# ray-project/ray

Measured on AMD Instinct MI355X. Metric: train_samples_per_sec, higher is better.
Workload: dtype bf16; 1 GPU; model=llama3-8b, global_batch=8, micro_batch=8, seq_len=4096, parallelism=dp1, n_params=8030261248, bucket_mb=128, grad_checkpoint=False, harness=ray_amd.train.TorchTrainer

## Files before the change

### __graft_entry__.py

```python
from __future__ import annotations

import os
import sys

sys.path.insert(0, os.path.dirname(os.path.abspath(__file__)))


def build() -> None:
    os.environ.setdefault("PYTORCH_ROCM_ARCH", "gfx950")
    from ray_amd.csrc import build as _b

    _b.build(verbose=True)
    import ray_amd
    import ray_amd.ops

    assert os.path.exists(_b.OUT), "HIP extension missing after build"


def smoke() -> None:
    import torch

    from ray_amd.models.llama import CONFIGS, LlamaModel
    from ray_amd.ops import HAVE_HIP_OPS, FusedAdamW

    assert torch.cuda.is_available(), "smoke() needs a GPU"
    assert HAVE_HIP_OPS, "ray_amd HIP extension not loaded"
    dev = torch.device("cuda", 0)
    cfg = CONFIGS["llama-tiny"]
    model = LlamaModel(cfg, dtype=torch.bfloat16).to(dev)
    model.cosT = model.cosT.to(dev)
    model.sinT = model.sinT.to(dev)
    tokens = torch.randint(0, cfg.vocab_size, (2, 128), device=dev)
    targets = torch.randint(0, cfg.vocab_size, (2, 128), device=dev)
    loss = model(tokens, targets)
    loss.backward()
    opt = FusedAdamW(model.parameters(), lr=1e-3)
    opt.step()
    torch.cuda.synchronize()
    print("smoke ok: loss", float(loss.detach().float().cpu()))


if __name__ == "__main__":
    build()
    if "--smoke" in sys.argv:
        smoke()
```

### ray_amd/csrc/ops.hip

```cpp
#include <torch/extension.h>
#include <ATen/hip/HIPContext.h>

#include "hip/rmsnorm.hip"
#include "hip/elementwise.hip"
#include "hip/rl_scans.hip"
#include "hip/cross_entropy.hip"
#include "hip/flash_attn_v5.hip"
#include "hip/flash_attn_v6.hip"
#include "hip/fa_bwd.hip"
#include "hip/fa_bwd_v3.hip"
#include "hip/fa_bwd_v4.hip"
#include "hip/fa_bwd_dq_v4.hip"
#include "hip/fa_bwd_dkv_v5.hip"
#include "hip/fa_bwd_dkv_v6.hip"
#include "hip/fa_bwd_dq_v5.hip"
#include "hip/gemv.hip"
#include "hip/paged_attn.hip"

#define CHECK_IN(x)                                                     \
  TORCH_CHECK(x.is_cuda(), #x " must be on GPU");                       \
  TORCH_CHECK(x.is_contiguous(), #x " must be contiguous")

static inline hipStream_t cur_stream() {
  return at::hip::getCurrentHIPStream().stream();
}

static inline int grid_for(long long n, int block = 256, int cap = 2048) {
  long long g = (n + block - 1) / block;
  return (int)std::min<long long>(g, cap);
}


std::vector<at::Tensor> rmsnorm_fwd(at::Tensor x, at::Tensor w, double eps) {
  CHECK_IN(x);
  CHECK_IN(w);
  TORCH_CHECK(x.scalar_type() == at::kBFloat16, "x must be bf16");
  int H = (int)x.size(-1);
  TORCH_CHECK(H % 8 == 0, "H must be a multiple of 8");
  long long N = x.numel() / H;
  auto y = at::empty_like(x);
  auto inv = at::empty({N}, x.options().dtype(at::kFloat));
  hipLaunchKernelGGL(rmsnorm_fwd_bf16, dim3((unsigned)N), dim3(256), 0,
                     cur_stream(), (const short*)x.data_ptr(),
                     (const short*)w.data_ptr(), (short*)y.data_ptr(),
                     inv.data_ptr<float>(), H, (float)eps);
  return {y, inv};
}

std::vector<at::Tensor> rmsnorm_bwd(at::Tensor dy, at::Tensor x, at::Tensor w,
                                    at::Tensor inv) {
  CHECK_IN(dy); CHECK_IN(x); CHECK_IN(w); CHECK_IN(inv);
  int H = (int)x.size(-1);
  long long N = x.numel() / H;
  auto dx = at::empty_like(x);
  auto dw = at::zeros({H}, x.options().dtype(at::kFloat));
  hipLaunchKernelGGL(rmsnorm_bwd_dx_bf16, dim3((unsigned)N), dim3(256), 0,
                     cur_stream(), (const short*)dy.data_ptr(),
                     (const short*)x.data_ptr(), (const short*)w.data_ptr(),
                     inv.data_ptr<float>(), (short*)dx.data_ptr(), H);
  int row_splits = (int)std::min<long long>(256, std::max<long long>(1, N / 64));
  hipLaunchKernelGGL(rmsnorm_bwd_dw_bf16,
                     dim3((H + 255) / 256, row_splits), dim3(256), 0,
                     cur_stream(), (const short*)dy.data_ptr(),
                     (const short*)x.data_ptr(), inv.data_ptr<float>(),
                     dw.data_ptr<float>(), N, H);
  return {dx, dw};
}


at::Tensor swiglu_fwd(at::Tensor a, at::Tensor b) {
  CHECK_IN(a); CHECK_IN(b);
  TORCH_CHECK(a.numel() == b.numel() && a.numel() % 8 == 0);
  auto y = at::empty_like(a);
  long long n8 = a.numel() / 8;
  hipLaunchKernelGGL(swiglu_fwd_bf16, dim3(grid_for(n8)), dim3(256), 0,
                     cur_stream(), (const short*)a.data_ptr(),
                     (const short*)b.data_ptr(), (short*)y.data_ptr(), n8);
  return y;
}

std::vector<at::Tensor> swiglu_bwd(at::Tensor dy, at::Tensor a, at::Tensor b) {
  CHECK_IN(dy); CHECK_IN(a); CHECK_IN(b);
  auto da = at::empty_like(a);
  auto db = at::empty_like(b);
  long long n8 = a.numel() / 8;
  hipLaunchKernelGGL(swiglu_bwd_bf16, dim3(grid_for(n8)), dim3(256), 0,
                     cur_stream(), (const short*)dy.data_ptr(),
                     (const short*)a.data_ptr(), (const short*)b.data_ptr(),
                     (short*)da.data_ptr(), (short*)db.data_ptr(), n8);
  return {da, db};
}


at::Tensor rope_apply(at::Tensor x, at::Tensor cosT, at::Tensor sinT,
                      int64_t n_heads, int64_t T, int64_t sign) {
  CHECK_IN(cosT); CHECK_IN(sinT);
  int D = (int)x.size(-1);
  long long rows = x.numel() / D;
  long long in_rs = (long long)n_heads * D;
  if (!x.is_contiguous()) {
// ... 120 lines not shown
              "paged_attn: num_splits must be 1..1024");
  auto out = at::empty({B, Hq, D}, q.options());
  at::Tensor ws;
  float *ws_o = nullptr, *ws_ml = nullptr;
  if (S > 1) {
    long long need = (long long)B * Hq * S * (D + 2);
    if (workspace.has_value()) {
      ws = *workspace;
      CHECK_IN(ws);
      TORCH_CHECK(ws.scalar_type() == at::kFloat && ws.numel() >= need,
                  "paged_attn: workspace must be fp32 with >= B*Hq*S*(D+2) "
                  "elements");
    } else {
      ws = at::empty({need}, q.options().dtype(at::kFloat));
    }
    ws_o = ws.data_ptr<float>();
    ws_ml = ws_o + (long long)B * Hq * S * D;
  }
#define PA_LAUNCH(DD, RR)                                                   \
  launch_paged_decode<DD, RR>(q, k_cache, v_cache, block_table, seq_lens,   \
                              out, ws_o, ws_ml, S, Hkv)
#define PA_REP(DD)                                                          \
  switch (rep) {                                                            \
    case 1: PA_LAUNCH(DD, 1); break;                                        \
    case 2: PA_LAUNCH(DD, 2); break;                                        \
    case 4: PA_LAUNCH(DD, 4); break;                                        \
    default: PA_LAUNCH(DD, 8); break;                                       \
  }
  if (D == 64) { PA_REP(64) } else { PA_REP(128) }
#undef PA_REP
#undef PA_LAUNCH
  if (S > 1) launch_paged_reduce(ws, out, B, Hq, D, S);
  return out;
}

static long long paged_row_stride(const at::Tensor& t, const char* name) {
  TORCH_CHECK(t.is_cuda(), name, " must be on GPU");
  TORCH_CHECK(t.scalar_type() == at::kBFloat16, name, " must be bf16");
  TORCH_CHECK(t.dim() == 3 && t.stride(2) == 1 && t.stride(1) == t.size(2),
              name, " must be [B, H, D] with a contiguous [H, D] tail");
  TORCH_CHECK(t.stride(0) % 8 == 0 &&
              reinterpret_cast<uintptr_t>(t.data_ptr()) % 16 == 0,
              name, " rows must be 16-byte aligned");
  return (long long)t.stride(0);
}

at::Tensor rope_append_paged(at::Tensor q, at::Tensor k, at::Tensor v,
                             at::Tensor cosT, at::Tensor sinT, at::Tensor pos,
                             at::Tensor block_table, at::Tensor k_cache,
                             at::Tensor v_cache) {
  long long q_rs = paged_row_stride(q, "q");
  long long k_rs = paged_row_stride(k, "k");
  long long v_rs = paged_row_stride(v, "v");
  CHECK_IN(cosT); CHECK_IN(sinT);
  CHECK_I32(pos);
  CHECK_I32(block_table);
  int B = (int)q.size(0), Hq = (int)q.size(1), D = (int)q.size(2);
  int Hkv = (int)k.size(1);
  TORCH_CHECK(D == 64 || D == 128, "paged_attn: head_dim must be 64 or 128");
  TORCH_CHECK(k.size(0) == B && v.size(0) == B && k.size(2) == D &&
              v.size(2) == D && v.size(1) == Hkv,
              "q/k/v shapes disagree");
  check_paged_cache(k_cache, v_cache, Hkv, D);
  TORCH_CHECK(cosT.scalar_type() == at::kFloat &&
              sinT.scalar_type() == at::kFloat && cosT.dim() == 2 &&
              cosT.size(1) == D / 2 && sinT.sizes() == cosT.sizes(),
              "cosT/sinT must be fp32 [T, D/2]");
  TORCH_CHECK(pos.dim() == 1 && pos.size(0) == B, "pos must be [B]");
  TORCH_CHECK(block_table.dim() == 2 && block_table.size(0) == B &&
              block_table.size(1) >= 1,
              "block_table must be [B, max_pages]");
  auto q_rot = at::empty({B, Hq, D}, q.options());
  if (B == 0) return q_rot;
  hipLaunchKernelGGL(rope_append_paged_bf16, dim3(B), dim3(256), 0,
                     cur_stream(), (const short*)q.data_ptr(),
                     (const short*)k.data_ptr(), (const short*)v.data_ptr(),
                     q_rs, k_rs, v_rs, cosT.data_ptr<float>(),
                     sinT.data_ptr<float>(), pos.data_ptr<int>(),
                     block_table.data_ptr<int>(), (short*)k_cache.data_ptr(),
                     (short*)v_cache.data_ptr(), (short*)q_rot.data_ptr(), Hq,
                     Hkv, D, (int)cosT.size(0), (int)k_cache.size(0),
                     (int)block_table.size(1));
  return q_rot;
}


void adamw_step(at::Tensor p, at::Tensor g, at::Tensor m, at::Tensor v,
                at::Tensor master, double lr, double beta1, double beta2,
                double eps, double wd, int64_t step, double grad_scale) {
  CHECK_IN(p); CHECK_IN(g); CHECK_IN(m); CHECK_IN(v);
  long long n = p.numel();
  float bc1 = 1.f - powf((float)beta1, (float)step);
  float bc2 = 1.f - powf((float)beta2, (float)step);
  if (p.scalar_type() == at::kBFloat16) {
    CHECK_IN(master);
    hipLaunchKernelGGL(adamw_step_bf16, dim3(grid_for(n)), dim3(256), 0,
                       cur_stream(), (short*)p.data_ptr(),
                       (const short*)g.data_ptr(), m.data_ptr<float>(),
                       v.data_ptr<float>(), master.data_ptr<float>(), n,
                       (float)lr, (float)beta1, (float)beta2, (float)eps,
                       (float)wd, bc1, bc2, (float)grad_scale);
  } else {
    hipLaunchKernelGGL(adamw_step_f32, dim3(grid_for(n)), dim3(256), 0,
                       cur_stream(), p.data_ptr<float>(),
                       g.data_ptr<float>(), m.data_ptr<float>(),
                       v.data_ptr<float>(), n, (float)lr, (float)beta1,
                       (float)beta2, (float)eps, (float)wd, bc1, bc2,
                       (float)grad_scale);
  }
}


std::vector<at::Tensor> gae(at::Tensor rewards, at::Tensor values,
                            at::Tensor cont, double gamma, double lam) {
  CHECK_IN(rewards); CHECK_IN(values); CHECK_IN(cont);
  int T = (int)rewards.size(0);
  int B = (int)rewards.size(1);
  TORCH_CHECK(values.size(0) == T + 1, "values must be [T+1, B]");
  auto adv = at::empty_like(rewards);
  auto vt = at::empty_like(rewards);
  hipLaunchKernelGGL(gae_scan_f32, dim3((B + 255) / 256), dim3(256), 0,
                     cur_stream(), rewards.data_ptr<float>(),
                     values.data_ptr<float>(), cont.data_ptr<float>(),
                     adv.data_ptr<float>(), vt.data_ptr<float>(), T, B,
                     (float)gamma, (float)lam);
  return {adv, vt};
}

std::vector<at::Tensor> vtrace(at::Tensor log_rhos, at::Tensor rewards,
                               at::Tensor values, at::Tensor cont,
                               double gamma, double rho_clip, double c_clip,
                               double rho_pg_clip) {
  CHECK_IN(log_rhos); CHECK_IN(rewards); CHECK_IN(values); CHECK_IN(cont);
  int T = (int)rewards.size(0);
  int B = (int)rewards.size(1);
  auto vs = at::empty_like(rewards);
  auto pg = at::empty_like(rewards);
  hipLaunchKernelGGL(vtrace_scan_f32, dim3((B + 255) / 256), dim3(256), 0,
                     cur_stream(), log_rhos.data_ptr<float>(),
                     rewards.data_ptr<float>(), values.data_ptr<float>(),
                     cont.data_ptr<float>(), vs.data_ptr<float>(),
                     pg.data_ptr<float>(), T, B, (float)gamma,
                     (float)rho_clip, (float)c_clip, (float)rho_pg_clip);
  return {vs, pg};
}


at::Tensor img_normalize(at::Tensor in, at::Tensor mean, at::Tensor inv_std) {
  CHECK_IN(in); CHECK_IN(mean); CHECK_IN(inv_std);
  TORCH_CHECK(in.scalar_type() == at::kByte && in.dim() == 4);
  long long N = in.size(0);
  int H = (int)in.size(1), W = (int)in.size(2), C = (int)in.size(3);
  auto out = at::empty({N, C, H, W}, in.options().dtype(at::kBFloat16));
  long long total = in.numel();
  hipLaunchKernelGGL(img_norm_u8_bf16, dim3(grid_for(total)), dim3(256), 0,
                     cur_stream(), in.data_ptr<unsigned char>(),
                     (short*)out.data_ptr(), mean.data_ptr<float>(),
                     inv_std.data_ptr<float>(), N, H, W, C);
  return out;
}


std::vector<at::Tensor> ce_fwd(at::Tensor logits, at::Tensor target) {
  CHECK_IN(logits); CHECK_IN(target);
  TORCH_CHECK(logits.scalar_type() == at::kBFloat16);
  TORCH_CHECK(target.scalar_type() == at::kInt);
// ... 165 lines not shown
    }
    if (v4 && getenv("RAY_AMD_FA_NO_DKV5") == nullptr) {
      hipLaunchKernelGGL(fa_bwd_dkv_v5_bf16, dim3(T / 256, B * Hkv),
                         dim3(512), 0, cur_stream(),
                         (const short*)q.data_ptr(),
                         (const short*)k.data_ptr(),
                         (const short*)v.data_ptr(),
                         (const short*)d_o.data_ptr(), lse.data_ptr<float>(),
                         dsum.data_ptr<float>(), (short*)dk.data_ptr(),
                         (short*)dv.data_ptr(), B, Hq, Hkv, T,
                         causal ? 1 : 0, scale, bthd);
      return {dq, dk, dv};
    }
    if (v4) {
      hipLaunchKernelGGL(fa_bwd_dv_v4_bf16, dim3(T / 256, B * Hkv),
                         dim3(512), 0, cur_stream(),
                         (const short*)q.data_ptr(),
                         (const short*)k.data_ptr(),
                         (const short*)v.data_ptr(),
                         (const short*)d_o.data_ptr(), lse.data_ptr<float>(),
                         (short*)dv.data_ptr(), B, Hq, Hkv, T,
                         causal ? 1 : 0, scale, bthd);
      hipLaunchKernelGGL(fa_bwd_dk_v4_bf16, dim3(T / 256, B * Hkv),
                         dim3(512), 0, cur_stream(),
                         (const short*)q.data_ptr(),
                         (const short*)k.data_ptr(),
                         (const short*)v.data_ptr(),
                         (const short*)d_o.data_ptr(), lse.data_ptr<float>(),
                         dsum.data_ptr<float>(), (short*)dk.data_ptr(), B,
                         Hq, Hkv, T, causal ? 1 : 0, scale, bthd);
      return {dq, dk, dv};
    }
    hipLaunchKernelGGL(fa_bwd_dv_v3_bf16, dim3(T / 128, B * Hkv),
                       dim3(256), 0, cur_stream(),
                       (const short*)q.data_ptr(),
                       (const short*)k.data_ptr(),
                       (const short*)v.data_ptr(),
                       (const short*)d_o.data_ptr(), lse.data_ptr<float>(),
                       (short*)dv.data_ptr(), B, Hq, Hkv, T,
                       causal ? 1 : 0, scale);
    hipLaunchKernelGGL(fa_bwd_dk_v3_bf16, dim3(T / 128, B * Hkv),
                       dim3(256), 0, cur_stream(),
                       (const short*)q.data_ptr(),
                       (const short*)k.data_ptr(),
                       (const short*)v.data_ptr(),
                       (const short*)d_o.data_ptr(), lse.data_ptr<float>(),
                       dsum.data_ptr<float>(), (short*)dk.data_ptr(), B,
                       Hq, Hkv, T, causal ? 1 : 0, scale);
    return {dq, dk, dv};
  }
  if (split) {
    hipLaunchKernelGGL(fa_bwd_dv_bf16, dim3(T / 128, B * Hkv), dim3(256),
                       0, cur_stream(), (const short*)q.data_ptr(),
                       (const short*)k.data_ptr(),
                       (const short*)v.data_ptr(),
                       (const short*)d_o.data_ptr(), lse.data_ptr<float>(),
                       (short*)dv.data_ptr(), B, Hq, Hkv, T,
                       causal ? 1 : 0, scale);
    hipLaunchKernelGGL(fa_bwd_dk_bf16, dim3(T / 128, B * Hkv), dim3(256),
                       0, cur_stream(), (const short*)q.data_ptr(),
                       (const short*)k.data_ptr(),
                       (const short*)v.data_ptr(),
                       (const short*)d_o.data_ptr(), lse.data_ptr<float>(),
                       dsum.data_ptr<float>(), (short*)dk.data_ptr(), B,
                       Hq, Hkv, T, causal ? 1 : 0, scale);
  } else {
    hipLaunchKernelGGL(fa_bwd_dkv_bf16, dim3(T / 128, B * Hkv), dim3(256),
                       0, cur_stream(), (const short*)q.data_ptr(),
                       (const short*)k.data_ptr(),
                       (const short*)v.data_ptr(),
                       (const short*)d_o.data_ptr(), lse.data_ptr<float>(),
                       dsum.data_ptr<float>(), (short*)dk.data_ptr(),
                       (short*)dv.data_ptr(), B, Hq, Hkv, T,
                       causal ? 1 : 0, scale);
  }
  return {dq, dk, dv};
}

PYBIND11_MODULE(TORCH_EXTENSION_NAME, m) {
  m.def("flash_attn_fwd", &flash_attn_fwd);
  m.def("flash_attn_bwd", &flash_attn_bwd);
  m.def("rmsnorm_fwd", &rmsnorm_fwd);
  m.def("gemv", &gemv);
  m.def("paged_attn_decode", &paged_attn_decode, py::arg("q"),
        py::arg("k_cache"), py::arg("v_cache"), py::arg("block_table"),
        py::arg("seq_lens"), py::arg("num_splits"),
        py::arg("workspace") = py::none());
  m.def("paged_attn_reduce", &paged_attn_reduce);
  m.def("rope_append_paged", &rope_append_paged);
  m.def("rmsnorm_bwd", &rmsnorm_bwd);
  m.def("swiglu_fwd", &swiglu_fwd);
  m.def("swiglu_bwd", &swiglu_bwd);
  m.def("rope_apply", &rope_apply);
  m.def("adamw_step", &adamw_step);
  m.def("gae", &gae);
  m.def("vtrace", &vtrace);
  m.def("img_normalize", &img_normalize);
  m.def("ce_fwd", &ce_fwd);
  m.def("ce_bwd", &ce_bwd);
  m.attr("gfx_arch") = "gfx950";
}
```

### ray_amd/models/llama.py

```python
from __future__ import annotations

from dataclasses import dataclass

import os

import torch
import torch.nn as nn
import torch.nn.functional as F

from ray_amd import ops


@dataclass
class LlamaConfig:
    vocab_size: int = 128256
    hidden_size: int = 4096
    intermediate_size: int = 14336
    num_layers: int = 32
    num_heads: int = 32
    num_kv_heads: int = 8
    max_seq_len: int = 8192
    rope_base: float = 500000.0
    rms_eps: float = 1e-5
    tie_embeddings: bool = False


CONFIGS = {
    "llama3-8b": LlamaConfig(),
    "llama3-1b": LlamaConfig(
        hidden_size=2048, intermediate_size=8192, num_layers=16,
        num_heads=32, num_kv_heads=8
    ),
    "llama-tiny": LlamaConfig(
        vocab_size=512, hidden_size=256, intermediate_size=512,
        num_layers=2, num_heads=4, num_kv_heads=2, max_seq_len=512,
    ),
}


class Attention(nn.Module):
    def __init__(self, cfg: LlamaConfig, dtype=torch.bfloat16):
        super().__init__()
        self.cfg = cfg
        self.head_dim = cfg.hidden_size // cfg.num_heads
        self.n_rep = cfg.num_heads // cfg.num_kv_heads
        self._fused_qkv = not os.environ.get("RAY_AMD_NO_FUSED_QKV")
        qd = cfg.num_heads * self.head_dim
        kvd = cfg.num_kv_heads * self.head_dim
        if self._fused_qkv:
            self.qkv_proj = nn.Linear(
                cfg.hidden_size, qd + 2 * kvd, bias=False, dtype=dtype
            )
        else:
            self.q_proj = nn.Linear(
                cfg.hidden_size, qd, bias=False, dtype=dtype)
            self.k_proj = nn.Linear(
                cfg.hidden_size, kvd, bias=False, dtype=dtype)
            self.v_proj = nn.Linear(
                cfg.hidden_size, kvd, bias=False, dtype=dtype)
        self.o_proj = nn.Linear(
            cfg.num_heads * self.head_dim, cfg.hidden_size, bias=False, dtype=dtype
        )

    def qkv(self, x, lin=None):
        B, T, _ = x.shape
        cfg = self.cfg
        hd = self.head_dim
        if self._fused_qkv:
            qkv = (self.qkv_proj(x) if lin is None
                   else lin(x, self.qkv_proj.weight))
            q, k, v = qkv.split(
                [cfg.num_heads * hd, cfg.num_kv_heads * hd,
                 cfg.num_kv_heads * hd], dim=-1)
            return (q.view(B, T, cfg.num_heads, hd),
                    k.view(B, T, cfg.num_kv_heads, hd),
                    v.view(B, T, cfg.num_kv_heads, hd))
        if lin is None:
            return (self.q_proj(x).view(B, T, cfg.num_heads, hd),
                    self.k_proj(x).view(B, T, cfg.num_kv_heads, hd),
                    self.v_proj(x).view(B, T, cfg.num_kv_heads, hd))
        return (lin(x, self.q_proj.weight).view(B, T, cfg.num_heads, hd),
                lin(x, self.k_proj.weight).view(B, T, cfg.num_kv_heads, hd),
                lin(x, self.v_proj.weight).view(B, T, cfg.num_kv_heads, hd))

    def forward(self, x, cosT, sinT, kv_cache=None, pos0: int = 0):
        B, T, H = x.shape
        cfg = self.cfg
        q, k, v = self.qkv(x)
        if self._fused_qkv:
            v = v.contiguous()
        q = ops.rope(q, cosT[pos0 : pos0 + T], sinT[pos0 : pos0 + T])
        k = ops.rope(k, cosT[pos0 : pos0 + T], sinT[pos0 : pos0 + T])
        q = q.transpose(1, 2)
        k = k.transpose(1, 2)
        v = v.transpose(1, 2)
        if kv_cache is not None:
            k, v = kv_cache.update(k, v, pos0)
        is_causal = kv_cache is None or T > 1
        if (
            kv_cache is None
            and q.is_cuda
            and q.dtype == torch.bfloat16
            and self.head_dim == 128
            and T % 128 == 0
            and not os.environ.get("RAY_AMD_ATTN_SDPA")
        ):
            out = ops.flash_attention(q, k, v, causal=True)
        else:
            out = F.scaled_dot_product_attention(
                q, k, v, is_causal=is_causal, enable_gqa=True
            )
        out = out.transpose(1, 2).reshape(B, T, -1)
        return self.o_proj(out)


class MLP(nn.Module):
    def __init__(self, cfg: LlamaConfig, dtype=torch.bfloat16):
        super().__init__()
        self.gate_proj = nn.Linear(
            cfg.hidden_size, cfg.intermediate_size, bias=False, dtype=dtype
        )
        self.up_proj = nn.Linear(
            cfg.hidden_size, cfg.intermediate_size, bias=False, dtype=dtype
        )
        self.down_proj = nn.Linear(
            cfg.intermediate_size, cfg.hidden_size, bias=False, dtype=dtype
        )

    def forward(self, x):
        return self.down_proj(ops.swiglu(self.gate_proj(x), self.up_proj(x)))


class Block(nn.Module):
    def __init__(self, cfg: LlamaConfig, dtype=torch.bfloat16):
        super().__init__()
        self.attn_norm = ops.RMSNorm(cfg.hidden_size, cfg.rms_eps, dtype)
        self.attn = Attention(cfg, dtype)
        self.mlp_norm = ops.RMSNorm(cfg.hidden_size, cfg.rms_eps, dtype)
        self.mlp = MLP(cfg, dtype)

    def forward(self, x, cosT, sinT, kv_cache=None, pos0=0):
        x = x + self.attn(self.attn_norm(x), cosT, sinT, kv_cache, pos0)
        x = x + self.mlp(self.mlp_norm(x))
        return x


class LlamaModel(nn.Module):
    def __init__(self, cfg: LlamaConfig, dtype=torch.bfloat16,
                 gradient_checkpointing: bool = False):
        super().__init__()
        self.cfg = cfg
        self.dtype = dtype
        self.embed = nn.Embedding(cfg.vocab_size, cfg.hidden_size, dtype=dtype)
        self.layers = nn.ModuleList(Block(cfg, dtype) for _ in range(cfg.num_layers))
        self.final_norm = ops.RMSNorm(cfg.hidden_size, cfg.rms_eps, dtype)
        self.lm_head = nn.Linear(
            cfg.hidden_size, cfg.vocab_size, bias=False, dtype=dtype
        )
        if cfg.tie_embeddings:
            self.lm_head.weight = self.embed.weight
        cosT, sinT = ops.rope_tables(
            cfg.max_seq_len, cfg.hidden_size // cfg.num_heads, cfg.rope_base
        )
        self.register_buffer("cosT", cosT, persistent=False)
        self.register_buffer("sinT", sinT, persistent=False)
        self.gradient_checkpointing = gradient_checkpointing
        self.apply(self._init_weights)

    def _init_weights(self, m):
        if isinstance(m, nn.Linear):
            nn.init.normal_(m.weight, std=0.02)
        elif isinstance(m, nn.Embedding):
            nn.init.normal_(m.weight, std=0.02)

    def forward(self, tokens, targets=None, kv_caches=None, pos0: int = 0):
        x = self.embed(tokens)
        for i, layer in enumerate(self.layers):
            cache = kv_caches[i] if kv_caches is not None else None
            if self.gradient_checkpointing and self.training:
                x = torch.utils.checkpoint.checkpoint(
                    layer, x, self.cosT, self.sinT, use_reentrant=False
                )
            else:
                x = layer(x, self.cosT, self.sinT, cache, pos0)
        x = self.final_norm(x)
        if targets is not None:
            if x.is_cuda and os.environ.get("RAY_AMD_CHUNKED_CE"):
                return ops.lm_head_cross_entropy(
                    x.reshape(-1, self.cfg.hidden_size),
                    self.lm_head.weight,
                    targets.reshape(-1),
                )
            logits = self.lm_head(x)
            return ops.cross_entropy(
                logits.view(-1, self.cfg.vocab_size), targets.reshape(-1)
            )
        return self.lm_head(x)

    def num_params(self) -> int:
        return sum(p.numel() for p in self.parameters())


class GraphedDecoder:

    def __init__(self, model: "LlamaModel", batch_size: int, max_T: int,
                 device):
        self.m = model
        cfg = model.cfg
        self.B = batch_size
        self.max_T = max_T
        self.device = device
        hd = cfg.hidden_size // cfg.num_heads
        dt = model.dtype
        self.cache_k = [
            torch.zeros(batch_size, cfg.num_kv_heads, max_T, hd,
                        device=device, dtype=dt)
            for _ in range(cfg.num_layers)
        ]
        self.cache_v = [torch.zeros_like(k) for k in self.cache_k]
        self.in_tok = torch.zeros(batch_size, 1, dtype=torch.long, device=device)
        self.pos = torch.zeros(1, dtype=torch.long, device=device)
        self.mask = torch.full((1, 1, 1, max_T), float("-inf"),
                               device=device, dtype=torch.float32)
        self.out_logits = None
        self.graph = None

    def _step(self):
        m = self.m
        cfg = m.cfg
        B = self.B
        hd = cfg.hidden_size // cfg.num_heads
        x = m.embed(self.in_tok)
        cos = m.cosT.index_select(0, self.pos).view(1, 1, 1, hd // 2)
        sin = m.sinT.index_select(0, self.pos).view(1, 1, 1, hd // 2)
        lin = ops.linear_sb
        for li, layer in enumerate(m.layers):
            h = layer.attn_norm(x)
            at = layer.attn
            q, k, v = at.qkv(h, lin=lin)
# ... 169 lines not shown
```

### ray_amd/ops/__init__.py

```python
from __future__ import annotations

import torch

try:
    from ray_amd import _hip_ops as _K

    HAVE_HIP_OPS = True
except ImportError:
    _K = None
    HAVE_HIP_OPS = False


def _require_ext(name: str):
    if _K is None:
        raise RuntimeError(
            f"ray_amd HIP extension not built but {name} was called on a GPU "
            "tensor. Run `python ray_amd/csrc/build.py`."
        )




def rmsnorm_ref(x: torch.Tensor, w: torch.Tensor, eps: float = 1e-5):
    xf = x.float()
    inv = torch.rsqrt(xf.pow(2).mean(-1, keepdim=True) + eps)
    return (xf * inv * w.float()).to(x.dtype)


class _RMSNorm(torch.autograd.Function):
    @staticmethod
    def forward(ctx, x, w, eps):
        _require_ext("rmsnorm")
        y, inv = _K.rmsnorm_fwd(x.contiguous(), w.contiguous(), eps)
        ctx.save_for_backward(x, w, inv)
        return y

    @staticmethod
    def backward(ctx, dy):
        x, w, inv = ctx.saved_tensors
        dx, dw = _K.rmsnorm_bwd(dy.contiguous(), x, w, inv)
        return dx, dw.to(w.dtype), None


def rmsnorm(x: torch.Tensor, w: torch.Tensor, eps: float = 1e-5):
    if not x.is_cuda:
        xf = x.float()
        inv = torch.rsqrt(xf.pow(2).mean(-1, keepdim=True) + eps)
        return (xf * inv * w.float()).to(x.dtype)
    return _RMSNorm.apply(x, w, eps)


class RMSNorm(torch.nn.Module):
    def __init__(self, dim: int, eps: float = 1e-5, dtype=torch.bfloat16):
        super().__init__()
        self.weight = torch.nn.Parameter(torch.ones(dim, dtype=dtype))
        self.eps = eps

    def forward(self, x):
        return rmsnorm(x, self.weight, self.eps)




def swiglu_ref(a: torch.Tensor, b: torch.Tensor):
    return (torch.nn.functional.silu(a.float()) * b.float()).to(a.dtype)


class _SwiGLU(torch.autograd.Function):
    @staticmethod
    def forward(ctx, a, b):
        _require_ext("swiglu")
        a = a.contiguous()
        b = b.contiguous()
        ctx.save_for_backward(a, b)
        return _K.swiglu_fwd(a, b)

    @staticmethod
    def backward(ctx, dy):
        a, b = ctx.saved_tensors
        da, db = _K.swiglu_bwd(dy.contiguous(), a, b)
        return da, db


def swiglu(a: torch.Tensor, b: torch.Tensor):
    if not a.is_cuda:
        return torch.nn.functional.silu(a) * b
    return _SwiGLU.apply(a, b)




def rope_tables(T: int, D: int, base: float = 500000.0, device="cpu"):
    half = D // 2
    inv_freq = 1.0 / (
        base ** (torch.arange(0, half, dtype=torch.float64) / half)
    )
    t = torch.arange(T, dtype=torch.float64)
    ang = torch.outer(t, inv_freq)
    return (
        ang.cos().float().contiguous().to(device),
        ang.sin().float().contiguous().to(device),
    )


def rope_ref(x: torch.Tensor, cosT: torch.Tensor, sinT: torch.Tensor):
    B, T, Hn, D = x.shape
    half = D // 2
    x1 = x[..., :half].float()
    x2 = x[..., half:].float()
    c = cosT[:T].view(1, T, 1, half)
    s = sinT[:T].view(1, T, 1, half)
    return torch.cat([x1 * c - x2 * s, x2 * c + x1 * s], dim=-1).to(x.dtype)


class _Rope(torch.autograd.Function):
    @staticmethod
    def forward(ctx, x, cosT, sinT, n_heads, T):
        _require_ext("rope")
        ctx.meta = (cosT, sinT, n_heads, T)
        if not (x.dim() == 4 and x.stride(3) == 1
                and x.stride(2) == x.size(3)
                and x.stride(0) == x.size(1) * x.stride(1)):
            x = x.contiguous()
        return _K.rope_apply(x, cosT, sinT, n_heads, T, 1)

    @staticmethod
    def backward(ctx, dy):
        cosT, sinT, n_heads, T = ctx.meta
        dx = _K.rope_apply(dy.contiguous(), cosT, sinT, n_heads, T, -1)
        return dx, None, None, None, None


def rope(x: torch.Tensor, cosT: torch.Tensor, sinT: torch.Tensor):
    B, T, Hn, D = x.shape
    if not x.is_cuda:
        return rope_ref(x, cosT, sinT)
    return _Rope.apply(x, cosT[:T].contiguous(), sinT[:T].contiguous(), Hn, T)


def linear_sb(x: torch.Tensor, weight: torch.Tensor) -> torch.Tensor:
    K = x.shape[-1]
    rows = x.numel() // K
    if (
        _K is not None
        and x.is_cuda
        and x.dtype == torch.bfloat16
        and weight.dtype == torch.bfloat16
        and rows <= 2
        and weight.shape[0] <= 8192
        and K % 512 == 0
        and not torch.is_grad_enabled()
    ):
        y = _K.gemv(x.reshape(rows, K).contiguous(), weight)
        return y.view(*x.shape[:-1], weight.shape[0])
    return torch.nn.functional.linear(x, weight)




def cross_entropy_ref(logits: torch.Tensor, target: torch.Tensor):
    return torch.nn.functional.cross_entropy(
        logits.float(), target.long(), ignore_index=-100, reduction="mean"
    )


class _FusedCE(torch.autograd.Function):
    @staticmethod
    def forward(ctx, logits, target):
        _require_ext("cross_entropy")
        logits = logits.contiguous()
        t32 = target.to(torch.int32).contiguous()
        loss, mx, lse = _K.ce_fwd(logits, t32)
        nvalid = (t32 >= 0).sum().clamp(min=1)
        ctx.save_for_backward(logits, t32, mx, lse, nvalid)
        return loss.sum() / nvalid.float()

    @staticmethod
    def backward(ctx, dloss):
        logits, t32, mx, lse, nvalid = ctx.saved_tensors
        per_row = (dloss / nvalid.float()).expand(logits.size(0)).contiguous()
        dl = _K.ce_bwd(logits, t32, mx, lse, per_row)
        return dl, None


def cross_entropy(logits: torch.Tensor, target: torch.Tensor):
    if not logits.is_cuda:
        return cross_entropy_ref(logits, target)
    return _FusedCE.apply(logits, target)


class _ChunkedLmHeadCE(torch.autograd.Function):

    @staticmethod
    def forward(ctx, x, weight, target, chunk_rows):
        _require_ext("cross_entropy")
        x = x.contiguous()
        t32 = target.to(torch.int32).contiguous()
        N = x.shape[0]
        nvalid = (t32 >= 0).sum().clamp(min=1)
        loss_sum = torch.zeros((), dtype=torch.float32, device=x.device)
        for s in range(0, N, chunk_rows):
            e = min(s + chunk_rows, N)
            logits = (x[s:e] @ weight.t()).contiguous()
            l, mx, lse = _K.ce_fwd(logits, t32[s:e])
            loss_sum += l.sum()
        ctx.save_for_backward(x, weight, t32, nvalid)
        ctx.chunk = chunk_rows
        return loss_sum / nvalid.float()

    @staticmethod
    def backward(ctx, dloss):
        x, w, t32, nvalid = ctx.saved_tensors
        N = x.shape[0]
        chunk = ctx.chunk
        dx = torch.empty_like(x)
        dw_acc = torch.zeros_like(w, dtype=torch.float32)
        scale = dloss / nvalid.float()
        for s in range(0, N, chunk):
            e = min(s + chunk, N)
            logits = (x[s:e] @ w.t()).contiguous()
            _, mx, lse = _K.ce_fwd(logits, t32[s:e])
            per_row = scale.expand(e - s).contiguous()
            dl = _K.ce_bwd(logits, t32[s:e], mx, lse, per_row)
            dx[s:e] = dl @ w
            dw_acc += (dl.t() @ x[s:e]).float()
        return dx, dw_acc.to(w.dtype), None, None


def lm_head_cross_entropy(x: torch.Tensor, weight: torch.Tensor,
                          target: torch.Tensor,
                          chunk_rows: int = 8192) -> torch.Tensor:
    if not x.is_cuda:
        return cross_entropy_ref(x.float() @ weight.t().float(), target)
    return _ChunkedLmHeadCE.apply(x, weight, target, chunk_rows)




# ... 315 lines not shown
```

Measured before the change: 4.818 samples/s.

## Add custom MFMA weight-gradient GEMM kernel and route Linear backward through it

Adds a hand-written HIP bf16 weight-gradient GEMM (dy^T @ x) with 256x256 output tiles, LDS double buffering via global_load_lds, transposed LDS reads, XCD-aware tile scheduling and an optional wave-stagger barrier. A custom autograd Linear routes backward dW through this kernel for a table of Llama-8B shapes. A grouped variant computes the gate and up projection weight gradients in a single launch. It aims to beat the library GEMM on the tall-skinny reduction-over-tokens shape, at the cost of extra launch-shape restrictions and a Python autograd layer around every projection.

```diff
diff --git a/__graft_entry__.py b/__graft_entry__.py
--- a/__graft_entry__.py
+++ b/__graft_entry__.py
@@ -36,6 +36,11 @@
     loss.backward()
     opt = FusedAdamW(model.parameters(), lr=1e-3)
     opt.step()
+    from ray_amd.ops import gemm_wgrad
+    dy = torch.randn(128, 256, device=dev).bfloat16()
+    x = torch.randn(128, 256, device=dev).bfloat16()
+    dw, ref = gemm_wgrad(dy, x).float(), dy.float().t() @ x.float()
+    assert (dw - ref).norm() <= 5e-3 * ref.norm(), "gemm_wgrad mismatch"
     torch.cuda.synchronize()
     print("smoke ok: loss", float(loss.detach().float().cpu()))
 
diff --git a/ray_amd/csrc/hip/gemm_wgrad.hip b/ray_amd/csrc/hip/gemm_wgrad.hip
--- /dev/null
+++ b/ray_amd/csrc/hip/gemm_wgrad.hip
@@ -0,0 +1,243 @@
+#include "common.h"
+#include "fa_bwd_lds_layout.h"
+
+typedef __attribute__((ext_vector_type(8))) __bf16 wg_bf16x8;
+typedef __attribute__((ext_vector_type(16))) float wg_f32x16;
+typedef __attribute__((ext_vector_type(2))) unsigned int wg_u32x2;
+typedef __attribute__((ext_vector_type(4))) unsigned int wg_u32x4;
+
+#define WG_STAGE 65536
+#define WG_HALF 16384
+#define WG_B 32768
+
+template <int OFF>
+DEV_INLINE wg_u32x2 wg_tr(unsigned addr) {
+  wg_u32x2 v;
+  asm volatile("ds_read_b64_tr_b16 %0, %1 offset:%2"
+               : "=v"(v)
+               : "v"(addr), "n"(OFF)
+               : "memory");
+  return v;
+}
+
+DEV_INLINE wg_bf16x8 wg_frag(wg_u32x2 lo, wg_u32x2 hi) {
+  wg_u32x4 t = __builtin_shufflevector(lo, hi, 0, 1, 2, 3);
+  return __builtin_bit_cast(wg_bf16x8, t);
+}
+
+DEV_INLINE void wg_stage_half(const char* g, unsigned lane_off, char* lds) {
+  typedef const __attribute__((address_space(1))) void* gptr;
+  typedef __attribute__((address_space(3))) void* lptr;
+  __builtin_amdgcn_global_load_lds((gptr)(g + lane_off), (lptr)lds, 16, 0, 0);
+  __builtin_amdgcn_global_load_lds((gptr)(g + 128 + lane_off),
+                                   (lptr)(lds + 1024), 16, 0, 0);
+}
+
+struct WgRegs {
+  wg_f32x16 acc[2][2][2];
+  wg_u32x2 a[2][4][2];
+  wg_u32x2 b[4][2];
+};
+
+template <int BASE, int S>
+DEV_INLINE void wg_read_a1(WgRegs& r, unsigned a0, unsigned a1) {
+  r.a[0][S][0] = wg_tr<BASE + 4096 * S>(a0);
+  r.a[0][S][1] = wg_tr<BASE + 4096 * S + 2048>(a1);
+  r.a[1][S][0] = wg_tr<BASE + 4096 * S + 512>(a0);
+  r.a[1][S][1] = wg_tr<BASE + 4096 * S + 2048 + 512>(a1);
+}
+template <int BASE>
+DEV_INLINE void wg_read_a(WgRegs& r, unsigned a0, unsigned a1) {
+  wg_read_a1<BASE, 0>(r, a0, a1);
+  wg_read_a1<BASE, 1>(r, a0, a1);
+  wg_read_a1<BASE, 2>(r, a0, a1);
+  wg_read_a1<BASE, 3>(r, a0, a1);
+}
+
+template <int BASE, int S>
+DEV_INLINE void wg_read_b1(WgRegs& r, unsigned b0, unsigned b1) {
+  r.b[S][0] = wg_tr<BASE + 4096 * S>(b0);
+  r.b[S][1] = wg_tr<BASE + 4096 * S + 2048>(b1);
+}
+template <int BASE>
+DEV_INLINE void wg_read_b(WgRegs& r, unsigned b0, unsigned b1) {
+  wg_read_b1<BASE, 0>(r, b0, b1);
+  wg_read_b1<BASE, 1>(r, b0, b1);
+  wg_read_b1<BASE, 2>(r, b0, b1);
+  wg_read_b1<BASE, 3>(r, b0, b1);
+}
+
+template <int HA, int HB>
+DEV_INLINE void wg_mma(WgRegs& r) {
+  asm volatile("s_waitcnt lgkmcnt(0)" ::: "memory");
+  __builtin_amdgcn_sched_barrier(0);
+  __builtin_amdgcn_s_barrier();
+  __builtin_amdgcn_sched_barrier(0);
+  __builtin_amdgcn_s_setprio(1);
+#pragma unroll
+  for (int s = 0; s < 4; ++s) {
+    const wg_bf16x8 bf = wg_frag(r.b[s][0], r.b[s][1]);
+#pragma unroll
+    for (int i = 0; i < 2; ++i)
+      r.acc[HA][HB][i] = __builtin_amdgcn_mfma_f32_32x32x16_bf16(
+          wg_frag(r.a[i][s][0], r.a[i][s][1]), bf, r.acc[HA][HB][i], 0, 0, 0);
+  }
+  __builtin_amdgcn_s_setprio(0);
+  __builtin_amdgcn_sched_barrier(0);
+  __builtin_amdgcn_s_barrier();
+  __builtin_amdgcn_sched_barrier(0);
+}
+
+template <int ST, bool NEXT_B0, bool NEXT2, int VMC>
+DEV_INLINE void wg_tile(WgRegs& r, const unsigned (&ra)[2][2],
+                        const unsigned (&rb)[2][2], char* lds_w, const char* gA,
+                        const char* gB, unsigned la, unsigned lb,
+                        long long tileA, long long tileB, int t) {
+  constexpr int S = ST * WG_STAGE;
+  constexpr int O = (ST ^ 1) * WG_STAGE;
+  wg_read_a<0>(r, ra[ST][0], ra[ST][1]);
+  wg_read_b<0>(r, rb[ST][0], rb[ST][1]);
+  if (NEXT_B0)
+    wg_stage_half(gB + (t + 1) * tileB, lb, lds_w + O + WG_B);
+  wg_mma<0, 0>(r);
+  wg_read_b<WG_HALF>(r, rb[ST][0], rb[ST][1]);
+  if (NEXT2) wg_stage_half(gA + (t + 2) * tileA, la, lds_w + S);
+  wg_mma<0, 1>(r);
+  wg_read_a<WG_HALF>(r, ra[ST][0], ra[ST][1]);
+  if (NEXT2)
+    wg_stage_half(gB + (t + 2) * tileB + 256, lb, lds_w + S + WG_B + WG_HALF);
+  wg_mma<1, 1>(r);
+  wg_read_b<0>(r, rb[ST][0], rb[ST][1]);
+  if (NEXT2)
+    wg_stage_half(gA + (t + 2) * tileA + 256, la, lds_w + S + WG_HALF);
+  if (VMC == 6) asm volatile("s_waitcnt vmcnt(6)" ::: "memory");
+  if (VMC == 0) asm volatile("s_waitcnt vmcnt(0)" ::: "memory");
+  wg_mma<1, 0>(r);
+}
+
+template <bool STAGGER>
+__global__ __launch_bounds__(512) void gemm_wgrad_bf16(
+    const short* __restrict__ dy0, const short* __restrict__ dy1,
+    const short* __restrict__ x, short* __restrict__ out0,
+    short* __restrict__ out1, int M, long long ldy, long long ldx,
+    long long ldo, int NT, int nt0, int KT) {
+  __shared__ __attribute__((aligned(1024))) char smem[2 * WG_STAGE];
+
+  const int tid = threadIdx.x;
+  const int w = __builtin_amdgcn_readfirstlane(tid >> 6);
+  const int lane = tid & 63;
+  const int wr = w >> 2, wc = w & 3;
+
+  int tn, tk;
+  {
+    const int nwg = NT * KT;
+    const int orig = blockIdx.x;
+    const int xcd = orig & 7;
+    const int q = nwg >> 3, rr = nwg & 7;
+    const int id = (xcd < rr ? xcd * (q + 1) : rr * (q + 1) + (xcd - rr) * q) +
+                   (orig >> 3);
+    const int per = 8 * KT;
+    const int grp = id / per;
+    const int first = grp * 8;
+    const int gsz = min(NT - first, 8);
+    const int in = id - grp * per;
+    tn = first + in % gsz;
+    tk = in / gsz;
+  }
+  const bool p1 = tn >= nt0;
+  const short* dy = p1 ? dy1 : dy0;
+  short* out = p1 ? out1 : out0;
+  const int tn_l = p1 ? tn - nt0 : tn;
+
+  const char* gA = reinterpret_cast<const char*>(dy + (long long)tn_l * 256);
+  const char* gB = reinterpret_cast<const char*>(x + (long long)tk * 256);
+  const long long tileA = 64 * ldy * 2, tileB = 64 * ldx * 2;
+
+  unsigned la, lb;
+  {
+    const int r7 = (lane >> 2) & 7;
+    const int xo = 2 * (w & 1) + (r7 >> 2);
+    const int ch = 4 * (lane >> 5) + ((lane & 3) ^ xo);
+    const int row = 8 * w + r7;
+    la = (unsigned)(row * (int)ldy * 2 + 16 * ch);
+    lb = (unsigned)(row * (int)ldx * 2 + 16 * ch);
+  }
+  char* const lds_w = smem + 2048 * w;
+
+  const unsigned sm0 = (unsigned)(size_t)(
+      (__attribute__((address_space(3))) char*)smem);
+  unsigned ra[2][2], rb[2][2];
+#pragma unroll
+  for (int mm = 0; mm < 2; ++mm) {
+    const unsigned tb = sm0 + 2 * fb6_tbase(lane, mm);
+    ra[0][mm] = tb + 1024 * wr;
+    ra[1][mm] = tb + 1024 * wr + WG_STAGE;
+    rb[0][mm] = tb + 512 * wc + WG_B;
+    rb[1][mm] = tb + 512 * wc + WG_B + WG_STAGE;
+  }
+
+  WgRegs r;
+#pragma unroll
+  for (int a = 0; a < 2; ++a)
+#pragma unroll
+    for (int b = 0; b < 2; ++b)
+#pragma unroll
+      for (int i = 0; i < 2; ++i) r.acc[a][b][i] = wg_f32x16{};
+
+  const int nt = M >> 6;
+
+  wg_stage_half(gA, la, lds_w);
+  wg_stage_half(gB, lb, lds_w + WG_B);
+  wg_stage_half(gB + 256, lb, lds_w + WG_B + WG_HALF);
+  wg_stage_half(gA + 256, la, lds_w + WG_HALF);
+  wg_stage_half(gA + tileA, la, lds_w + WG_STAGE);
+  wg_stage_half(gB + tileB + 256, lb, lds_w + WG_STAGE + WG_B + WG_HALF);
+  wg_stage_half(gA + tileA + 256, la, lds_w + WG_STAGE + WG_HALF);
+  asm volatile("s_waitcnt vmcnt(6)" ::: "memory");
+  __builtin_amdgcn_s_barrier();
+  __builtin_amdgcn_sched_barrier(0);
+  if (STAGGER && wr) __builtin_amdgcn_s_barrier();
+  __builtin_amdgcn_sched_barrier(0);
+
+  int t = 0;
+  for (; t < nt - 2; t += 2) {
+    wg_tile<0, true, true, 6>(r, ra, rb, lds_w, gA, gB, la, lb, tileA, tileB,
+                              t);
+    wg_tile<1, true, true, 6>(r, ra, rb, lds_w, gA, gB, la, lb, tileA, tileB,
+                              t + 1);
+  }
+  wg_tile<0, true, false, 0>(r, ra, rb, lds_w, gA, gB, la, lb, tileA, tileB,
+                             t);
+  wg_tile<1, false, false, -1>(r, ra, rb, lds_w, gA, gB, la, lb, tileA, tileB,
+                               t + 1);
+  if (STAGGER && !wr) __builtin_amdgcn_s_barrier();
+  __builtin_amdgcn_sched_barrier(0);
+
+  short* const ep = reinterpret_cast<short*>(smem);
+  const int hi = lane >> 5, c32 = lane & 31;
+#pragma unroll
+  for (int ha = 0; ha < 2; ++ha) {
+#pragma unroll
+    for (int hb = 0; hb < 2; ++hb)
+#pragma unroll
+      for (int i = 0; i < 2; ++i)
+#pragma unroll
+        for (int g = 0; g < 16; ++g) {
+          const int row = 64 * wr + 32 * i + (g & 3) + 8 * (g >> 2) + 4 * hi;
+          const int col = 128 * hb + 32 * wc + c32;
+          ep[row * 256 + col] =
+              __builtin_bit_cast(short, (__bf16)r.acc[ha][hb][i][g]);
+        }
+    __syncthreads();
+#pragma unroll
+    for (int it = 0; it < 8; ++it) {
+      const int c = tid + 512 * it;
+      const int row = c >> 5, ch = c & 31;
+      const short8 v = *reinterpret_cast<const short8*>(ep + row * 256 + 8 * ch);
+      *reinterpret_cast<short8*>(
+          out + ((long long)tn_l * 256 + 128 * ha + row) * ldo +
+          (long long)tk * 256 + 8 * ch) = v;
+    }
+    __syncthreads();
+  }
+}
diff --git a/ray_amd/csrc/ops.hip b/ray_amd/csrc/ops.hip
--- a/ray_amd/csrc/ops.hip
+++ b/ray_amd/csrc/ops.hip
@@ -16,6 +16,7 @@
 #include "hip/fa_bwd_dq_v5.hip"
 #include "hip/gemv.hip"
 #include "hip/paged_attn.hip"
+#include "hip/gemm_wgrad.hip"
 
 #define CHECK_IN(x)                                                     \
   TORCH_CHECK(x.is_cuda(), #x " must be on GPU");                       \
@@ -302,6 +303,78 @@
                      Hkv, D, (int)cosT.size(0), (int)k_cache.size(0),
                      (int)block_table.size(1));
   return q_rot;
+}
+
+
+static long long wgrad_operand(const at::Tensor& t, const char* name) {
+  TORCH_CHECK(t.is_cuda(), name, " must be on GPU");
+  TORCH_CHECK(t.scalar_type() == at::kBFloat16, name, " must be bf16");
+  TORCH_CHECK(t.dim() == 2 && t.stride(1) == 1 && t.stride(0) >= t.size(1),
+              name, " must be 2-D with unit column stride");
+  TORCH_CHECK(t.stride(0) % 8 == 0 &&
+              reinterpret_cast<uintptr_t>(t.data_ptr()) % 16 == 0,
+              name, " rows must be 16-byte aligned");
+  TORCH_CHECK(t.size(1) % 256 == 0 && t.size(1) >= 256, name,
+              ": columns must be a multiple of 256");
+  return (long long)t.stride(0);
+}
+
+static void launch_wgrad(const at::Tensor& dy0, const at::Tensor& dy1,
+                         const at::Tensor& x, at::Tensor& out0,
+                         at::Tensor& out1, int problems) {
+  const long long ldy = wgrad_operand(dy0, "dy");
+  const long long ldx = wgrad_operand(x, "x");
+  const long long ldo = wgrad_operand(out0, "out");
+  const long long M = dy0.size(0), N = dy0.size(1), K = x.size(1);
+  TORCH_CHECK(x.size(0) == M && M >= 128 && M % 128 == 0,
+              "gemm_wgrad: dy and x need the same number of rows, a "
+              "multiple of 128");
+  TORCH_CHECK(out0.size(0) == N && out0.size(1) == K,
+              "gemm_wgrad: out must be [N, K]");
+  TORCH_CHECK(ldy * 64 < (1ll << 30) && ldx * 64 < (1ll << 30),
+              "gemm_wgrad: row stride too large");
+  if (problems == 2) {
+    TORCH_CHECK(wgrad_operand(dy1, "dy1") == ldy && dy1.size(0) == M &&
+                    dy1.size(1) == N,
+                "gemm_wgrad: grouped dy operands must match");
+    TORCH_CHECK(wgrad_operand(out1, "out1") == ldo && out1.size(0) == N &&
+                    out1.size(1) == K,
+                "gemm_wgrad: grouped outputs must match");
+  }
+  const int nt0 = (int)(N / 256), KT = (int)(K / 256);
+  const int NT = nt0 * problems;
+  TORCH_CHECK((long long)NT * KT < (1ll << 31), "gemm_wgrad: grid too large");
+#define WGRAD_LAUNCH(ST)                                                     \
+  hipLaunchKernelGGL(gemm_wgrad_bf16<ST>, dim3((unsigned)(NT * KT)),         \
+                     dim3(512), 0, cur_stream(),                             \
+                     (const short*)dy0.data_ptr(),                           \
+                     (const short*)dy1.data_ptr(),                           \
+                     (const short*)x.data_ptr(), (short*)out0.data_ptr(),    \
+                     (short*)out1.data_ptr(), (int)M, ldy, ldx, ldo, NT,     \
+                     nt0, KT)
+  if (getenv("RAY_AMD_WGRAD_NO_STAGGER") != nullptr) {
+    WGRAD_LAUNCH(false);
+  } else {
+    WGRAD_LAUNCH(true);
+  }
+#undef WGRAD_LAUNCH
+}
+
+at::Tensor gemm_wgrad(at::Tensor dy, at::Tensor x,
+                      c10::optional<at::Tensor> out) {
+  at::Tensor o = out.has_value()
+                     ? *out
+                     : at::empty({dy.size(1), x.size(1)}, dy.options());
+  launch_wgrad(dy, dy, x, o, o, 1);
+  return o;
+}
+
+std::vector<at::Tensor> gemm_wgrad_grouped(at::Tensor dy0, at::Tensor dy1,
+                                           at::Tensor x) {
+  auto o0 = at::empty({dy0.size(1), x.size(1)}, dy0.options());
+  auto o1 = at::empty_like(o0);
+  launch_wgrad(dy0, dy1, x, o0, o1, 2);
+  return {o0, o1};
 }
 
 
@@ -633,6 +706,9 @@
   m.def("flash_attn_bwd", &flash_attn_bwd);
   m.def("rmsnorm_fwd", &rmsnorm_fwd);
   m.def("gemv", &gemv);
+  m.def("gemm_wgrad", &gemm_wgrad, py::arg("dy"), py::arg("x"),
+        py::arg("out") = py::none());
+  m.def("gemm_wgrad_grouped", &gemm_wgrad_grouped);
   m.def("paged_attn_decode", &paged_attn_decode, py::arg("q"),
         py::arg("k_cache"), py::arg("v_cache"), py::arg("block_table"),
         py::arg("seq_lens"), py::arg("num_splits"),
diff --git a/ray_amd/models/llama.py b/ray_amd/models/llama.py
--- a/ray_amd/models/llama.py
+++ b/ray_amd/models/llama.py
@@ -48,17 +48,17 @@
         qd = cfg.num_heads * self.head_dim
         kvd = cfg.num_kv_heads * self.head_dim
         if self._fused_qkv:
-            self.qkv_proj = nn.Linear(
+            self.qkv_proj = ops.Linear(
                 cfg.hidden_size, qd + 2 * kvd, bias=False, dtype=dtype
             )
         else:
-            self.q_proj = nn.Linear(
+            self.q_proj = ops.Linear(
                 cfg.hidden_size, qd, bias=False, dtype=dtype)
-            self.k_proj = nn.Linear(
+            self.k_proj = ops.Linear(
                 cfg.hidden_size, kvd, bias=False, dtype=dtype)
-            self.v_proj = nn.Linear(
+            self.v_proj = ops.Linear(
                 cfg.hidden_size, kvd, bias=False, dtype=dtype)
-        self.o_proj = nn.Linear(
+        self.o_proj = ops.Linear(
             cfg.num_heads * self.head_dim, cfg.hidden_size, bias=False, dtype=dtype
         )
 
@@ -117,18 +117,20 @@
 class MLP(nn.Module):
     def __init__(self, cfg: LlamaConfig, dtype=torch.bfloat16):
         super().__init__()
-        self.gate_proj = nn.Linear(
+        self.gate_proj = ops.Linear(
             cfg.hidden_size, cfg.intermediate_size, bias=False, dtype=dtype
         )
-        self.up_proj = nn.Linear(
+        self.up_proj = ops.Linear(
             cfg.hidden_size, cfg.intermediate_size, bias=False, dtype=dtype
         )
-        self.down_proj = nn.Linear(
+        self.down_proj = ops.Linear(
             cfg.intermediate_size, cfg.hidden_size, bias=False, dtype=dtype
         )
 
     def forward(self, x):
-        return self.down_proj(ops.swiglu(self.gate_proj(x), self.up_proj(x)))
+        gate, up = ops.swiglu_mlp_in(
+            x, self.gate_proj.weight, self.up_proj.weight)
+        return self.down_proj(ops.swiglu(gate, up))
 
 
 class Block(nn.Module):
@@ -154,7 +156,7 @@
         self.embed = nn.Embedding(cfg.vocab_size, cfg.hidden_size, dtype=dtype)
         self.layers = nn.ModuleList(Block(cfg, dtype) for _ in range(cfg.num_layers))
         self.final_norm = ops.RMSNorm(cfg.hidden_size, cfg.rms_eps, dtype)
-        self.lm_head = nn.Linear(
+        self.lm_head = ops.Linear(
             cfg.hidden_size, cfg.vocab_size, bias=False, dtype=dtype
         )
         if cfg.tie_embeddings:
diff --git a/ray_amd/ops/__init__.py b/ray_amd/ops/__init__.py
--- a/ray_amd/ops/__init__.py
+++ b/ray_amd/ops/__init__.py
@@ -1,4 +1,6 @@
 from __future__ import annotations
+
+import os
 
 import torch
 
@@ -154,6 +156,156 @@
         y = _K.gemv(x.reshape(rows, K).contiguous(), weight)
         return y.view(*x.shape[:-1], weight.shape[0])
     return torch.nn.functional.linear(x, weight)
+
+
+
+WGRAD_M_GRANULE = 128
+
+_WGRAD_TABLE: dict = {
+    (14336, 4096, 1): True,
+    (4096, 14336, 1): True,
+    (14336, 4096, 2): True,
+    (4096, 4096, 1): True,
+    (128256, 4096, 1): True,
+}
+
+_WGRAD_FORCE = False
+
+
+def _wgrad_switch_on() -> bool:
+    return not os.environ.get("RAY_AMD_NO_WGRAD_GEMM")
+
+
+def _wgrad_listed(N: int, K: int, problems: int = 1) -> bool:
+    if N % 256 or K % 256:
+        return False
+    return _WGRAD_FORCE or (N, K, problems) in _WGRAD_TABLE
+
+
+def _wgrad_operand_ok(t: torch.Tensor) -> bool:
+    return (t.is_cuda and t.dtype == torch.bfloat16 and t.dim() == 2
+            and t.stride(1) == 1 and t.stride(0) % 8 == 0
+            and t.stride(0) >= t.shape[1] and t.data_ptr() % 16 == 0
+            and t.shape[1] % 256 == 0 and t.shape[1] > 0
+            and t.stride(0) * 64 < 2 ** 30)
+
+
+def _wgrad_rows_ok(M: int) -> bool:
+    return M >= WGRAD_M_GRANULE and M % WGRAD_M_GRANULE == 0
+
+
+def gemm_wgrad(dy: torch.Tensor, x: torch.Tensor, out=None) -> torch.Tensor:
+    _require_ext("gemm_wgrad")
+    if not (_wgrad_operand_ok(dy) and _wgrad_operand_ok(x)
+            and dy.shape[0] == x.shape[0] and _wgrad_rows_ok(dy.shape[0])):
+        raise ValueError(
+            "gemm_wgrad: needs bf16 GPU operands [M,N], [M,K] with M % 128 "
+            "== 0, N % 256 == 0, K % 256 == 0 and 16-byte-aligned rows")
+    if out is not None and not (_wgrad_operand_ok(out) and tuple(out.shape)
+                                == (dy.shape[1], x.shape[1])):
+        raise ValueError("gemm_wgrad: out must be a bf16 [N,K] GPU tensor "
+                         "with 16-byte-aligned rows")
+    return _K.gemm_wgrad(dy, x, out)
+
+
+def gemm_wgrad_grouped(dy0: torch.Tensor, dy1: torch.Tensor,
+                       x: torch.Tensor):
+    _require_ext("gemm_wgrad")
+    if not (_wgrad_operand_ok(dy0) and _wgrad_operand_ok(dy1)
+            and _wgrad_operand_ok(x) and dy0.shape == dy1.shape
+            and dy0.stride(0) == dy1.stride(0)
+            and dy0.shape[0] == x.shape[0] and _wgrad_rows_ok(x.shape[0])):
+        raise ValueError("gemm_wgrad_grouped: operands do not qualify")
+    o0, o1 = _K.gemm_wgrad_grouped(dy0, dy1, x)
+    return o0, o1
+
+
+def _wgrad_use_kernel(dy2, x2, problems=1) -> bool:
+    return (_K is not None and _wgrad_switch_on()
+            and _wgrad_listed(dy2.shape[1], x2.shape[1], problems)
+            and _wgrad_operand_ok(dy2) and _wgrad_operand_ok(x2)
+            and _wgrad_rows_ok(dy2.shape[0]))
+
+
+def _wgrad(dy2: torch.Tensor, x2: torch.Tensor) -> torch.Tensor:
+    if _wgrad_use_kernel(dy2, x2):
+        return _K.gemm_wgrad(dy2, x2, None)
+    return dy2.t() @ x2
+
+
+class _LinearFn(torch.autograd.Function):
+    @staticmethod
+    def forward(ctx, x, weight):
+        ctx.save_for_backward(x, weight)
+        return torch.nn.functional.linear(x, weight)
+
+    @staticmethod
+    def backward(ctx, dy):
+        x, weight = ctx.saved_tensors
+        dx = dw = None
+        if ctx.needs_input_grad[0]:
+            dx = dy @ weight
+        if ctx.needs_input_grad[1]:
+            dw = _wgrad(dy.reshape(-1, dy.shape[-1]),
+                        x.reshape(-1, x.shape[-1]))
+        return dx, dw
+
+
+def _linear_custom(x, weight, bias=None) -> bool:
+    return (bias is None and x.is_cuda and weight.is_cuda
+            and x.dtype == torch.bfloat16 and weight.dtype == torch.bfloat16
+            and weight.dim() == 2 and torch.is_grad_enabled()
+            and _wgrad_switch_on())
+
+
+def linear(x: torch.Tensor, weight: torch.Tensor, bias=None) -> torch.Tensor:
+    if _linear_custom(x, weight, bias) and _wgrad_listed(*weight.shape):
+        return _LinearFn.apply(x, weight)
+    return torch.nn.functional.linear(x, weight, bias)
+
+
+class Linear(torch.nn.Linear):
+
+    def forward(self, x):
+        return linear(x, self.weight, self.bias)
+
+
+class _SwigluMlpIn(torch.autograd.Function):
+
+    @staticmethod
+    def forward(ctx, x, w_gate, w_up):
+        ctx.save_for_backward(x, w_gate, w_up)
+        return (torch.nn.functional.linear(x, w_gate),
+                torch.nn.functional.linear(x, w_up))
+
+    @staticmethod
+    def backward(ctx, d_gate, d_up):
+        x, w_gate, w_up = ctx.saved_tensors
+        dg2 = d_gate.reshape(-1, d_gate.shape[-1])
+        du2 = d_up.reshape(-1, d_up.shape[-1])
+        x2 = x.reshape(-1, x.shape[-1])
+        dx = dwg = dwu = None
+        if ctx.needs_input_grad[0]:
+            dx = (dg2 @ w_gate + du2 @ w_up).view(x.shape)
+        need_g, need_u = ctx.needs_input_grad[1], ctx.needs_input_grad[2]
+        if (need_g and need_u and dg2.stride() == du2.stride()
+                and _wgrad_use_kernel(dg2, x2, 2)
+                and _wgrad_operand_ok(du2)):
+            dwg, dwu = _K.gemm_wgrad_grouped(dg2, du2, x2)
+        else:
+            if need_g:
+                dwg = _wgrad(dg2, x2)
+            if need_u:
+                dwu = _wgrad(du2, x2)
+        return dx, dwg, dwu
+
+
+def swiglu_mlp_in(x: torch.Tensor, w_gate: torch.Tensor,
+                  w_up: torch.Tensor):
+    if (_linear_custom(x, w_gate) and _linear_custom(x, w_up)
+            and w_gate.shape == w_up.shape):
+        return _SwigluMlpIn.apply(x, w_gate, w_up)
+    return linear(x, w_gate), linear(x, w_up)
 
 
 
```

New measurement: 5.035 samples/s (median of 6 runs). 4.5% higher.
